# ajzhai/PEANUT

Hardware: AMD Instinct MI355X
Metric: maps/sec for 480x480x(4+N_cat) prediction fwd, batch 32 (higher is better)
Workload: dtype f32; 1 GPU; 480x480, 14-channel (4+10) partial maps -> 6-class prediction forward (PSPNet R50-V1c-D8), batch 32 per GPU, seeded random-init weights; survey_config=2, global_batch=32, parallelism=dp1 (map shards, no data-path collective)

## Files before the change

peanut_amd/csrc/options.h:

```cpp
#pragma once
#include <stdlib.h>
#include <string.h>

#include <string>

namespace peanut {

enum OptionId {
  OPT_PW_GLDS, OPT_PW256_MINK, OPT_PW256_MINTILES, OPT_PW256_PHASE, OPT_PW256_SKIP_PAD, OPT_PW256W_MINK, OPT_PW256W_MINTILES, OPT_PW256P_MINK, OPT_PW256P_MINTILES, OPT_PW256P_FLUSH, OPT_PW256P_ORDER, OPT_PW256P_STREAMK, OPT_PW256WP_MINK, OPT_PW256WP_MINTILES, OPT_PW256WP_NPRE, OPT_PW256WP_STAGGER, OPT_PW_ARES, OPT_PW_SKINNY,
  OPT_PW_ARES_MINUNITS, OPT_PATCH_MINTILES, OPT_STEM_NCHW, OPT_BN64_MAXK, OPT_PW_BN64_MAXK, OPT_PW64_MAXTILES, OPT_FP32_BK, OPT_NCHUNK, OPT_RES_PREFETCH, OPT_SPLIT_MODEL,
  OPT_RS_CONV, OPT_RS_BN64_MAXK, OPT_RS256_MINK, OPT_RS256_MINTILES, OPT_RS64_MAXK, OPT_RS64_MAXTILES,
  OPT_WINO_M, OPT_WINO_HEAD_M, OPT_WINO6_MAXDIL, OPT_WINO5_MINDIL, OPT_WINO_FLUSH_CH, OPT_WINO_MIN_CIN, OPT_WINO_NARROW_MINPIX, OPT_WINO_SMALL_MAXWG, OPT_DEFER_SPLITK,
  OPT_PPM_OVERLAP, OPT_PPM_GROUPED, OPT_PPM_TERM_ROWS, OPT_PPM_GROUP_ROWS, OPT_RCNN_WINO_M, OPT_RCNN_STEM_S2D, OPT_RCNN_RPN_FUSED, OPT_RCNN_FPN_OVERLAP, OPT_RCNN_RANK_SORT, OPT_RCNN_TOPK_SLICE, OPT_RCNN_NMS_LEVELS, OPT_FMM_LOCAL32, OPT_FMM_MAX_PASSES, OPT_FMM_BLOCKED, OPT_FMM_INNER,
  OPT_COUNT
};

struct OptionInfo {
  const char* key;
  long long def;
  bool upload_time;
  const char* help;
};

inline const OptionInfo* option_table() {
  static const OptionInfo t[OPT_COUNT] = {
      {"pw_glds", 1, false, "fp32 1x1 convs / grouped GEMMs on the LDS-DMA kernels of conv_pw.hip (0: conv_igemm)"},
      {"pw256_mink", 1024, false, "fewest input channels for the 256 x 128 three-stage kernel"},
      {"pw256_mintiles", 256, false, "fewest 256 x 128 tiles for that kernel"},
      {"pw256_phase", 1, false, "the two waves of a SIMD request their LDS-DMA pieces half an iteration apart"},
      {"pw256_skip_pad", 1, false, "256 x 128 kernel, grouped GEMMs: waves whose rows are all group padding issue no MFMAs (0: compute the zero rows)"},
      {"pw256w_mink", 768, false, "fewest input channels for the 256 x 256 two-stage kernel (0: off)"},
      {"pw256w_mintiles", 1536, false, "fewest 256 x 256 tiles for that kernel"},
      {"pw256p_mink", 512, false, "fewest input channels for the persistent 256 x 128 kernel (conv_pw256p.hip; 0: off)"},
      {"pw256p_mintiles", 512, false, "fewest 256 x 128 tiles for that kernel"},
      {"pw256p_flush", 512, false, "most input channels of a Winograd position GEMM (two-level accumulation) that runs on the persistent kernel (0: none)"},
      {"pw256p_order", 1, false, "persistent 256 x 128 kernel: 1 = the workgroups of an XCD walk its run of tiles side by side (neighbours share operand panels in L2), 0 = one contiguous run per workgroup"},
      {"pw256p_streamk", 1, false, "persistent 256 x 128 kernel: the tail tiles' k-tiles as one stream in equal runs per workgroup (0: every tail tile cut into the same number of parts)"},
      {"pw256wp_mink", 512, false, "fewest input channels for the persistent 256 x 256 kernel (conv_pw256wp.hip; 0: off)"},
      {"pw256wp_mintiles", 768, false, "fewest 256 x 256 tiles for that kernel"},
      {"pw256wp_npre", 0, false, "persistent 256 x 256 kernel: accumulator blocks per in-place epilogue group (2 or 4; 0 = two with a residual, four without)"},
      {"pw256wp_stagger", 0, false, "persistent 256 x 256 kernel: spread of the workgroups' start times in sleeps of ~3.4 us (their tile boundaries -- 512 KiB of epilogue traffic per CU -- then fall at different times)"},
      {"pw_ares", 1, false, "K = 128 / 256 pointwise layers on the persistent A-resident kernel (conv_pw_ares.hip)"},
      {"pw_skinny", 1, false, "grouped pointwise launches with at most 64 data rows per group (the PSP pyramid's per-scale convs and Q tables at batch 1) on the skinny weight-streaming kernel (gemm_skinny.hip: 6 KiB of LDS, fits next to any other kernel; 0: the MFMA kernels on 128-row padded tiles)"},
      {"pw_ares_minunits", 512, false, "fewest (m-tile, n-tile) units for that kernel"},
      {"patch_mintiles", 1024, false, "3x3 convs of 16 / 32 input channels on the persistent LDS-patch kernel (conv_patch.hip) from this many 8 x 16 output tiles (0: off)"},
      {"stem_nchw", 1, false, "prediction forward: the first stem conv reads the NCHW input itself (conv_patch.hip, NCHW variant) instead of a layout pass + NHWC conv (fp32 mode, when the patch kernel takes the layer)"},
      {"bn64_maxk", 256, true, "128 x 64 tiles for layers with at most this many input channels"},
      {"pw_bn64_maxk", 128, true, "pointwise layers / Winograd position GEMMs: weights PACKED 64 wide up to this many input channels (wider layers: 128-wide packing, 64-wide tiles chosen per shape)"},
      {"pw64_maxtiles", 512, false, "a 128-wide-packed pointwise layer with at most bn64_maxk input channels runs 128 x 64 tiles while its 128 x 128 tiling has fewer tiles than this (two per CU)"},
      {"fp32_bk", 0, true, "16: force 16-channel k-tiles in conv_igemm (experiment)"},
      {"nchunk", 8, false, "n-tiles per chunk of the tile order (0: n fastest over all n-tiles)"},
      {"res_prefetch", 1, false, "request the first residual rows before the last k-tile's MFMAs"},
      {"split_model", 1, false, "tail split-K plan counts CUs (1) or resident slots (0)"},
      {"rs_conv", 1, true, "emulated modes: non-pointwise convs on conv_rs.hip (0: fp32 MFMA kernel)"},
      {"rs_bn64_maxk", 128, true, "emulated modes: 128 x 64 tiles up to this many input channels"},
      {"rs256_mink", 512, false, "emulated modes: fewest input channels for the 256 x 256 kernel"},
      {"rs256_mintiles", 256, false, "emulated modes: fewest 256 x 256 tiles for it"},
      {"rs64_maxk", 512, false, "emulated modes: 64 x 64 tiles up to this many input channels"},
      {"rs64_maxtiles", 128, false, "emulated modes: ... and below this many 128-row tiles"},
      {"wino_m", 0, true, "4 / 5 / 6: force one Winograd form on every eligible layer (0: policy)"},
      {"wino_head_m", 0, true, "4 / 5 / 6: Winograd form of the PSP bottleneck (0: policy)"},
      {"wino6_maxdil", 4, true, "largest dilation that gets an F(6x6) form"},
      {"wino5_mindil", 4, true, "smallest dilation that also gets an F(5x5) form (0: none)"},
      {"wino_flush_ch", 64, true, "channels per partial sum of the position GEMMs' two-level accumulation (0: off)"},
      {"wino_min_cin", 0, true, "fewest input channels of a Winograd layer (0: the planner's policy)"},
      {"wino_narrow_minpix", 20000, false, "layers under 128 channels take their Winograd form from this many input pixels on (round 6: 100 000 -> 20 000 -- with the small-problem transforms one 720 x 720 map's layer1 conv2, 32 400 pixels, gains 5 us per layer as F(6x6); profiles/r9e)"},
      {"wino_small_maxwg", 1024, false, "Winograd transforms: launches with fewer workgroups than this of the one-thread-per-tile kernels take the small-problem variants (a workgroup per tile and 64-channel slice, a thread per line, through LDS; bit-identical; 0: never)"},
      {"defer_splitk", 1, false, "a Bottleneck conv1 whose every tile is split along k leaves its partial tiles unsummed and conv2's (small-problem) Winograd input transform sums them: one launch fewer per block at batch 1, bit-identical (0: every conv runs its own reduce); read when a (B, H, W) plan is built"},
      {"ppm_overlap", -1, false, "pyramid branch of the PSP head on a side stream: 0 / 1, -1 = by size"},
      {"ppm_grouped", -1, false, "per-scale PSP GEMMs as one grouped launch: 0 / 1, -1 = by size"},
      {"ppm_term_rows", 1, false, "folded pyramid term: one wave per output row, no barrier in the row loop (0: the workgroup-wide two-phase kernel)"},
      {"ppm_group_rows", 0, false, "pyramid pooling, row pass: rows added up per workgroup (1..5; 0 = by size: as many as still leave ~768 workgroups)"},
      {"rcnn_wino_m", 0, true, "detector front end: 4 / 5 / 6 pins one Winograd form (0: per shape)"},
      {"rcnn_stem_s2d", 1, true, "detector stem 7x7 stride 2 as a space-to-depth 4x4 conv"},
      {"rcnn_rpn_fused", 1, false, "detector: the RPN head on all five pyramid levels as one chain (five input transforms, ONE grouped Winograd GEMM, five output transforms, one objectness and one anchor-delta GEMM over all levels' rows: 12 launches instead of 25); read when a (B, H, W) plan is built"},
      {"rcnn_fpn_overlap", 0, false, "detector: the FPN output convs of p5, p4, p3 on a side stream next to the lateral / top-down chain that ends in p2's (round 5 experiment, bit-identical; measured SLOWER at batch 1, 5.70 against 5.61 ms per frame, profiles/r8: off); read when a (B, H, W) plan is built"},
      {"rcnn_rank_sort", 1, false, "detector: the RPN candidates of an image are ordered by counting the larger keys (n / 64 workgroups) instead of one workgroup's bitonic sort (round 5; same order: the keys are distinct)"},
      {"rcnn_topk_slice", 20480, false, "detector: objectness logits per workgroup of the per-level top-k (a level is cut into up to 8 ranges whose k largest are merged by counting; 0: one workgroup per level, round 4)"},
      {"rcnn_nms_levels", 1, false, "detector: the proposal NMS level by level (five 16 x 16-word suppression blocks and five scans per image side by side, post-NMS top-k by counting) instead of one score-sorted list per image (round 5; same proposals)"},
      {"fmm_local32", 1, false, "goal solver: single-precision local solve inside a tile"},
      {"fmm_max_passes", 24, false, "goal solver: hard ceiling of the second-order ordering passes; they stop as soon as a pass changes nothing (6-10 passes on the agent's 960 x 960 map; peanut_goal_converged reports whether they reached their fixed point)"},
      {"fmm_blocked", 1, false, "goal solver: a wave relaxes its 8 x 8 block of the tile to convergence between workgroup barriers (round 5; 0: one Jacobi sweep of the whole tile per barrier pair)"},
      {"fmm_inner", 48, false, "goal solver: iterations a wave spends on its block before it publishes it (blocked rounds)"},
  };
  return t;
}

struct Options {
  long long v[OPT_COUNT];
};

inline int option_index(const char* key) {
  if (!key) return -1;
  std::string k(key);
  for (auto& c : k) c = (char)((c >= 'A' && c <= 'Z') ? c - 'A' + 'a' : c);
  if (k.rfind("peanut_", 0) == 0) k = k.substr(7);
  const OptionInfo* t = option_table();
  for (int i = 0; i < OPT_COUNT; ++i)
    if (k == t[i].key) return i;
  return -1;
}

inline Options& default_options() {
  static Options d = [] {
    Options o;
    const OptionInfo* t = option_table();
    for (int i = 0; i < OPT_COUNT; ++i) {
      o.v[i] = t[i].def;
      std::string env = "PEANUT_";
      for (const char* c = t[i].key; *c; ++c) env += (char)((*c >= 'a' && *c <= 'z') ? *c - 'a' + 'A' : *c);
      const char* e = getenv(env.c_str());
      if (e && *e) o.v[i] = atoll(e);
    }
    return o;
  }();
  return d;
}

inline const Options*& active_options_ptr() {
  static thread_local const Options* p = nullptr;
  return p;
}

inline long long opt(OptionId id) {
  const Options* a = active_options_ptr();
  return (a ? a : &default_options())->v[id];
}

struct OptionScope {
  const Options* saved;
  explicit OptionScope(const Options* o) : saved(active_options_ptr()) { active_options_ptr() = o; }
  ~OptionScope() { active_options_ptr() = saved; }
  OptionScope(const OptionScope&) = delete;
  OptionScope& operator=(const OptionScope&) = delete;
};

}
```

peanut_amd/csrc/pred_api.hip:

```cpp
#include <math.h>
#include <string.h>

#include <map>
#include <memory>
#include <string>
#include <vector>

#include "net_common.h"

namespace peanut {

static thread_local std::string g_err;
void set_error(const std::string& msg) { g_err = msg; }
int fail(int code, const std::string& msg) {
  g_err = msg;
  return code;
}
static thread_local const char* g_kernel = "";
void note_kernel(const char* family) { g_kernel = family; }
const char* noted_kernel() { return g_kernel; }

namespace {

enum OpKind { OP_TO_NHWC, OP_CONV, OP_CONV_NCHW, OP_MAXPOOL, OP_PPM_POOL, OP_PPM_UP, OP_PPM_TERM, OP_UPSAMPLE, OP_WINO_IN, OP_WINO_GEMM, OP_WINO_OUT };

struct Op {
  OpKind kind;
  std::string name;
  std::string kernel;
  const ConvLayer* conv = nullptr;
  Act in, in2, res, out;
  bool has_in2 = false, has_res = false;
  double flops = 0;
  double bytes = 0;
  int wino_mt_per_group = 0;
  int wino_valid_rows = 0;
  int wino_gran = 128;
  int branch = 0;
  bool fork_before = false, join_before = false;
  int group_mt = 0;
  int ppm_scale_rows = 0;
  bool defer_ok = false;
};

struct Plan {
  int B = 0, H = 0, W = 0;
  Act splitk;
  Act splitk2;
  bool keep_all = false;
  size_t bytes = 0;
  std::vector<Op> ops;
  std::map<std::string, Act> named;
};

}
}

using namespace peanut;

struct peanut_conv {
  Options opts = default_options();
  ConvLayer L;
  DevBuf ws;
  DevBuf wino_v, wino_m;
};

struct peanut_pred {
  Options opts = default_options();
  DeferredSplit deferred{};
  peanut_pred_cfg cfg{};
  int cin_pad = 0;
  std::vector<std::unique_ptr<ConvLayer>> convs;
  ConvLayer* stem[3] = {nullptr, nullptr, nullptr};
  struct Block { ConvLayer *c1, *c2, *c3, *down, *c3d; };
  std::vector<std::vector<Block>> layers;
  std::vector<ConvLayer*> ppm;
  ConvLayer* bottleneck = nullptr;
  ConvLayer* bottleneck_x = nullptr;
  std::vector<ConvLayer*> ppm_q;
  std::unique_ptr<ConvLayer> ppm_grouped, ppmq_grouped;
  ConvLayer* conv_seg = nullptr;
  int feat_channels = 0;
  bool keep_all = false;
  std::map<std::string, std::unique_ptr<Plan>> plans;
  Plan* last_plan = nullptr;
  DevBuf ws;
  bool use_graph = false;
  GraphCache graphs;
  bool probe = false;
  Plan* probe_plan = nullptr;
  std::vector<std::vector<hipEvent_t>> probe_events;
  std::vector<hipEvent_t> event_pool;
  hipStream_t side = nullptr;
  hipEvent_t ev_fork = nullptr, ev_join = nullptr;
  ~peanut_pred() {
    for (auto& v : probe_events) for (auto e : v) (void)hipEventDestroy(e);
    for (auto e : event_pool) (void)hipEventDestroy(e);
    if (ev_fork) (void)hipEventDestroy(ev_fork);
    if (ev_join) (void)hipEventDestroy(ev_join);
    if (side) (void)hipStreamDestroy(side);
  }
};

namespace {

int bn_fold(peanut_pred* h, const TensorMap& tm, const std::string& bn, int cout, float* scale, float* shift) {
  return bn_fold_eps(tm, bn, cout, h->cfg.bn_eps, scale, shift);
}

int add_conv(peanut_pred* h, const TensorMap& tm, const std::string& conv, const std::string& bn, int cin,
             int cin_pad, int cout, int k, int stride, int pad, int dil, int relu, ConvLayer** out) {
  int rc = 0;
  const int64_t wshape[4] = {cout, cin, k, k};
  const peanut_tensor* w = tm.get(conv + ".weight", 4, wshape, &rc);
  if (!w) return rc;
  std::vector<float> scale(cout, 1.f), shift(cout, 0.f);
  const int64_t cshape[1] = {cout};
  if (!bn.empty()) {
    if ((rc = bn_fold(h, tm, bn, cout, scale.data(), shift.data()))) return rc;
  } else {
    const peanut_tensor* b = tm.get(conv + ".bias", 1, cshape, &rc); if (!b) return rc;
    for (int n = 0; n < cout; ++n) shift[n] = b->data[n];
  }
  auto L = std::make_unique<ConvLayer>();
  L->name = conv;
  rc = upload_conv(*L, w->data, scale.data(), shift.data(), cout, cin, cin_pad, k, k, stride, pad, dil, relu,
                   h->cfg.precision);
  if (rc) return rc;
  if (h->cfg.conv_algo == PEANUT_ALGO_AUTO && wino_eligible(cin_pad, cout, k, k, stride, pad, dil, h->cfg.precision, 64) &&
      (rc = upload_wino_forms(*L, w->data, scale.data(), shift.data(), cout, cin, cin_pad, pad, dil, relu, h->cfg.precision, 0)))
    return rc;
  *out = L.get();
  h->convs.push_back(std::move(L));
  return 0;
}

int add_fused_c3d(peanut_pred* h, const TensorMap& tm, const std::string& blk, int planes, int inplanes, int cout, ConvLayer** out) {
  int rc = 0;
  const int64_t w3s[4] = {cout, planes, 1, 1}, wds[4] = {cout, inplanes, 1, 1};
  const peanut_tensor* w3 = tm.get(blk + ".conv3.weight", 4, w3s, &rc);
  if (!w3) return rc;
  const peanut_tensor* wd = tm.get(blk + ".downsample.0.weight", 4, wds, &rc);
  if (!wd) return rc;
  std::vector<float> s3(cout), b3(cout), sd(cout), bd(cout);
  if ((rc = bn_fold(h, tm, blk + ".bn3", cout, s3.data(), b3.data()))) return rc;
  if ((rc = bn_fold(h, tm, blk + ".downsample.1", cout, sd.data(), bd.data()))) return rc;
  const int cin = planes + inplanes;
  std::vector<float> w((size_t)cout * cin), shift(cout);
  for (int n = 0; n < cout; ++n) {
    for (int c = 0; c < planes; ++c) w[(size_t)n * cin + c] = s3[n] * w3->data[(size_t)n * planes + c];
    for (int c = 0; c < inplanes; ++c) w[(size_t)n * cin + planes + c] = sd[n] * wd->data[(size_t)n * inplanes + c];
    shift[n] = b3[n] + bd[n];
  }
  auto L = std::make_unique<ConvLayer>();
  L->name = blk + ".conv3+downsample";
  if ((rc = upload_conv(*L, w.data(), nullptr, shift.data(), cout, cin, cin, 1, 1, 1, 0, 1, 1,
                        rs_planes_of(h->cfg.precision) ? h->cfg.precision : PEANUT_PREC_FP32))) return rc;
  *out = L.get();
  h->convs.push_back(std::move(L));
  return 0;
}

std::unique_ptr<ConvLayer> build_grouped(const std::vector<ConvLayer*>& parts, const std::string& name, int* rc) {
  *rc = 0;
  if (parts.size() < 2) return nullptr;
  const ConvDesc& d0 = parts[0]->d;
  for (const ConvLayer* L : parts)
    if (L->d.kh != 1 || L->d.kw != 1 || L->d.cin != d0.cin || L->d.cout != d0.cout || L->d.bn_tile != d0.bn_tile ||
        L->d.bk != d0.bk || L->d.relu != d0.relu || L->w.bytes != parts[0]->w.bytes || L->ss.bytes != parts[0]->ss.bytes)
      return nullptr;
  auto G = std::make_unique<ConvLayer>();
  G->name = name;
  G->d = d0;
  G->cin_real = parts[0]->cin_real;
  const size_t wb = parts[0]->w.bytes, sb = (size_t)d0.cout_pad * sizeof(float), n = parts.size();
// ... 119 lines not shown
      pl->ops.push_back(op);
    } else {
      push_conv(*pl, h->stem[i], x, nullptr, nullptr, y);
    }
    pl->named["stem" + std::to_string(i)] = y;
    if (!(i == 0 && nchw_stem)) rel(x);
    x = y;
  }
  {
    Act y = make_act(ar, B, conv_out_dim(x.H, 3, 2, 1, 1), conv_out_dim(x.W, 3, 2, 1, 1), x.C);
    Op op; op.kind = OP_MAXPOOL; op.name = "maxpool"; op.kernel = "maxpool"; op.in = x; op.out = y;
    op.bytes = (double)x.bytes + (double)y.bytes;
    pl->ops.push_back(op);
    pl->named["pool"] = y;
    rel(x);
    x = y;
  }
  for (size_t li = 0; li < h->layers.size(); ++li) {
    for (size_t bi = 0; bi < h->layers[li].size(); ++bi) {
      const auto& blk = h->layers[li][bi];
      const ConvDesc& d2 = blk.c2->d;
      Act t1 = make_act(ar, B, x.H, x.W, blk.c1->d.cout);
      push_conv(*pl, blk.c1, x, nullptr, nullptr, t1);
      const int h2 = conv_out_dim(x.H, 3, d2.stride, d2.pad, d2.dil), w2 = conv_out_dim(x.W, 3, d2.stride, d2.pad, d2.dil);
      Act t2 = make_act(ar, B, h2, w2, d2.cout);
      const size_t c1_idx = pl->ops.size() - 1;
      push_conv(*pl, blk.c2, t1, nullptr, nullptr, t2, &ar);
      {
        const Op& win = pl->ops[c1_idx + 1];
        if (opt(OPT_DEFER_SPLITK) != 0 && !h->keep_all && win.kind == OP_WINO_IN && pl->ops[c1_idx].kind == OP_CONV && !win.conv->d.rs &&
            wino_input_accepts_deferred(t1.B, t1.H, t1.W, t1.C, win.conv->d.dil, win.wino_gran, win.conv->wino_m))
          pl->ops[c1_idx].defer_ok = true;
      }
      rel(t1);
      Act idn = x;
      bool own_idn = false;
      const bool fused_c3d = blk.c3d != nullptr && !h->keep_all;
      if (blk.down && !fused_c3d) {
        idn = make_act(ar, B, h2, w2, blk.down->d.cout);
        push_conv(*pl, blk.down, x, nullptr, nullptr, idn);
        own_idn = true;
      }
      Act y = make_act(ar, B, h2, w2, blk.c3->d.cout);
      if (fused_c3d) push_conv(*pl, blk.c3d, t2, &x, nullptr, y);
      else push_conv(*pl, blk.c3, t2, nullptr, &idn, y);
      rel(t2);
      if (own_idn) rel(idn);
      rel(x);
      x = y;
    }
    pl->named["layer" + std::to_string(li + 1)] = x;
  }
  const int overlap_env = (int)opt(OPT_PPM_OVERLAP);
  const bool overlap = h->bottleneck_x != nullptr && (overlap_env >= 0 ? overlap_env == 1 : (long long)B * x.H * x.W >= 4096);
  const size_t side_first = pl->ops.size();
  if (overlap) {
    pl->splitk2.bytes = kSplitKScratchFloats * sizeof(float);
    pl->splitk2.off = ar.alloc(pl->splitk2.bytes);
    pl->splitk2.B = pl->splitk2.H = pl->splitk2.W = 1; pl->splitk2.C = 0;
  }
  std::vector<Act> side_bufs;
  auto rel_side = [&](const Act& t) { if (overlap) side_bufs.push_back(t); else rel(t); };
  int nbins = 0, kmax = 0;
  for (int i = 0; i < h->cfg.n_pool_scales; ++i) {
    nbins += h->cfg.pool_scales[i] * h->cfg.pool_scales[i];
    kmax = std::max(kmax, h->cfg.pool_scales[i]);
  }
  int srows = 0;
  if (h->ppm_grouped && h->ppmq_grouped && !h->keep_all) {
    const int cand = (B * kmax * kmax + 127) / 128 * 128;
    long long separate = 0;
    for (int i = 0; i < h->cfg.n_pool_scales; ++i) separate += ((long long)B * h->cfg.pool_scales[i] * h->cfg.pool_scales[i] + 127) / 128 * 128;
    const int env = (int)opt(OPT_PPM_GROUPED);
    if (env != 0 && ((long long)h->cfg.n_pool_scales * cand <= 2 * separate || env == 1)) srows = cand;
  }
  const int prow = srows ? h->cfg.n_pool_scales * srows : nbins * B;
  Act pooled = make_act(ar, 1, 1, prow, x.C);
  {
    Op op; op.kind = OP_PPM_POOL; op.name = "ppm_pool"; op.kernel = "ppm_pool"; op.in = x; op.out = pooled; op.ppm_scale_rows = srows;
    op.bytes = (double)x.bytes + (double)pooled.bytes;
    const size_t sf = ppm_pool_scratch_floats(B, x.H, x.C, h->cfg.pool_scales, h->cfg.n_pool_scales);
    if (sf) {
      Act scr; scr.B = 1; scr.H = 1; scr.W = 1; scr.C = 0; scr.bytes = sf * sizeof(float); scr.off = ar.alloc(scr.bytes);
      op.in2 = scr; op.has_in2 = true;
      pl->ops.push_back(op);
      rel_side(scr);
    } else {
      pl->ops.push_back(op);
    }
  }
  Act table = make_act(ar, 1, 1, prow, h->cfg.head_channels);
  auto push_grouped = [&](const ConvLayer* G, const Act& in, const Act& out) {
    push_conv(*pl, G, in, nullptr, nullptr, out);
    Op& op = pl->ops.back();
    op.group_mt = srows / 128;
    op.flops = 2.0 * (double)prow * G->d.cout * G->cin_real;
  };
  if (srows) {
    push_grouped(h->ppm_grouped.get(), pooled, table);
  } else {
    size_t row0 = 0;
    for (int i = 0; i < h->cfg.n_pool_scales; ++i) {
      const int k = h->cfg.pool_scales[i];
      Act in = pooled, out = table;
      in.off = pooled.off + row0 * (size_t)x.C * sizeof(float);
      in.H = 1; in.W = k * k; in.C = x.C; in.B = B;
      out.off = table.off + row0 * (size_t)h->cfg.head_channels * sizeof(float);
      out.H = 1; out.W = k * k; out.C = h->cfg.head_channels; out.B = B;
      push_conv(*pl, h->ppm[i], in, nullptr, nullptr, out);
      row0 += (size_t)B * k * k;
    }
  }
  pl->named["ppm_table"] = table;
  rel_side(pooled);
  Act bt;
  int term_scale_rows = 0;
  if (h->bottleneck_x) {
    const int hc = h->cfg.head_channels;
    Act q = make_act(ar, 1, 1, prow, 9 * hc);
    if (srows) {
      push_grouped(h->ppmq_grouped.get(), table, q);
      term_scale_rows = srows;
    } else {
      size_t row0 = 0;
      for (int i = 0; i < h->cfg.n_pool_scales; ++i) {
        const int k = h->cfg.pool_scales[i];
        Act in = table, out = q;
        in.off = table.off + row0 * (size_t)hc * sizeof(float);
        in.H = 1; in.W = k * k; in.C = hc; in.B = B;
        out.off = q.off + row0 * (size_t)(9 * hc) * sizeof(float);
        out.H = 1; out.W = k * k; out.C = 9 * hc; out.B = B;
        push_conv(*pl, h->ppm_q[i], in, nullptr, nullptr, out);
        row0 += (size_t)B * k * k;
      }
    }
    rel_side(table);
    Act r = make_act(ar, B, x.H, x.W, hc);
    {
      Op op; op.kind = OP_PPM_TERM; op.name = "ppm_conv_term"; op.kernel = "ppm_conv_term"; op.in = q; op.out = r; op.ppm_scale_rows = term_scale_rows;
      op.bytes = (double)q.bytes + (double)r.bytes;
      pl->ops.push_back(op);
    }
    rel_side(q);
    const size_t side_end = pl->ops.size();
    bt = make_act(ar, B, x.H, x.W, h->bottleneck_x->d.cout);
    push_conv(*pl, h->bottleneck_x, x, nullptr, &r, bt, &ar);
    if (overlap) {
      for (size_t i = side_first; i < side_end; ++i) pl->ops[i].branch = 1;
      pl->ops[side_first].fork_before = true;
      for (size_t i = side_end; i < pl->ops.size(); ++i)
        if (pl->ops[i].has_res) { pl->ops[i].join_before = true; break; }
      for (const auto& t : side_bufs) rel(t);
    }
    for (size_t i = side_first; i < side_end; ++i) {
      Op& op = pl->ops[i];
      if (op.kind == OP_CONV && op.group_mt == 1 && opt(OPT_PW_SKINNY) != 0 && B * kmax * kmax <= 64 &&
          op.conv->d.bn_tile == 128 && op.conv->d.bk == 32 && op.conv->d.cout % 128 == 0 && (op.conv->d.cin / 32) % 4 == 0)
        op.kernel = "gemm_skinny";
    }
    rel(r);
  } else {
    Act up = make_act(ar, B, x.H, x.W, h->cfg.n_pool_scales * h->cfg.head_channels);
    { Op op; op.kind = OP_PPM_UP; op.name = "ppm_upsample_concat"; op.kernel = "ppm_upsample_concat"; op.in = table; op.out = up; pl->ops.push_back(op); }
    rel(table);
    bt = make_act(ar, B, x.H, x.W, h->bottleneck->d.cout);
    push_conv(*pl, h->bottleneck, x, &up, nullptr, bt);
    rel(up);
  }
  pl->named["bottleneck"] = bt;
  rel(x);
  Act lo = make_act(ar, B, bt.H, bt.W, h->conv_seg->d.cout);
  push_conv(*pl, h->conv_seg, bt, nullptr, nullptr, lo);
  pl->named["logits_lowres"] = lo;
  rel(bt);
  {
    Op op; op.kind = OP_UPSAMPLE; op.name = "upsample_logits"; op.kernel = "upsample_logits"; op.in = lo;
    op.bytes = (double)lo.bytes + (double)B * H * W * h->conv_seg->d.cout * 4.0;
    pl->ops.push_back(op);
  }
  rel(lo);
  return pl;
}

}

static size_t plan_high_water(const Plan& pl) {
  size_t hw = 0;
  auto upd = [&](const Act& a) { if (a.bytes && a.off + Arena::round_up(a.bytes) > hw) hw = a.off + Arena::round_up(a.bytes); };
  for (const auto& op : pl.ops) {
    upd(op.in); upd(op.in2); upd(op.res); upd(op.out);
  }
  for (const auto& kv : pl.named) upd(kv.second);
  upd(pl.splitk);
  upd(pl.splitk2);
  return hw;
}

static Plan* get_plan(peanut_pred* h, int B, int H, int W) {
  if (B <= 0 || H < 16 || W < 16) { set_error("forward: need B >= 1 and H, W >= 16"); return nullptr; }
  const std::string key = std::to_string(B) + "x" + std::to_string(H) + "x" + std::to_string(W) + (h->keep_all ? "k" : "");
  auto it = h->plans.find(key);
  if (it == h->plans.end()) {
    auto pl = build_plan(h, B, H, W);
    pl->bytes = plan_high_water(*pl);
    it = h->plans.emplace(key, std::move(pl)).first;
  }
  return it->second.get();
}

static int run_op(peanut_pred* h, const Plan& pl, const Op& op, const float* in_dev, float* out_dev, int sigmoid,
                  hipStream_t s) {
  char* base = (char*)h->ws.p;
  auto P = [&](const Act& a) { return (float*)(base + a.off); };
  switch (op.kind) {
    case OP_TO_NHWC:
      return launch_nchw_to_nhwc_pad(in_dev, P(op.out), pl.B, h->cfg.in_channels, pl.H, pl.W, h->cin_pad, s);
    case OP_CONV_NCHW:
      return launch_conv_patch_nchw(op.conv->d, in_dev, h->cfg.in_channels, P(op.out), pl.B, pl.H, pl.W, op.out.H, op.out.W, s);
    case OP_CONV: {
      ConvArgs a{};
      a.x = P(op.in);
      a.x2 = op.has_in2 ? P(op.in2) : nullptr;
      a.res = op.has_res ? P(op.res) : nullptr;
      a.y = P(op.out);
      a.B = op.in.B; a.H = op.in.H; a.W = op.in.W;
      a.c1 = op.in.C; a.c2 = op.has_in2 ? op.in2.C : 0;
      a.Ho = op.out.H; a.Wo = op.out.W;
      a.ws = P(op.branch ? pl.splitk2 : pl.splitk); a.ws_floats = kSplitKScratchFloats;
      int scale_rows[8] = {0};
      if (op.group_mt) {
        int most = 0;
        for (int i = 0; i < h->cfg.n_pool_scales && i < 8; ++i) {
          scale_rows[i] = pl.B * h->cfg.pool_scales[i] * h->cfg.pool_scales[i];
          most = std::max(most, scale_rows[i]);
        }
        a.group_valid_rows = most;
        a.group_rows = scale_rows;
        a.mt_per_group = op.group_mt;
        a.w_group_stride = op.conv->w.bytes / sizeof(float) / (size_t)h->cfg.n_pool_scales;
        a.ss_group_stride = op.conv->d.cout_pad;
      }
      if (op.defer_ok) a.defer = &h->deferred;
      return launch_conv(op.conv->d, a, s);
    }
    case OP_WINO_IN: {
      const int rc = launch_wino_input(P(op.in), P(op.out), op.in.B, op.in.H, op.in.W, op.in.C, op.conv->d.dil, s, op.wino_gran, op.conv->wino_m, 0,
                                       h->deferred.valid ? &h->deferred : nullptr);
      h->deferred.valid = false;
      return rc;
    }
    case OP_WINO_GEMM: {
      ConvArgs a{};
      a.x = P(op.in); a.y = P(op.out);
      a.B = 1; a.H = 1; a.W = op.in.W; a.c1 = op.in.C; a.c2 = 0; a.Ho = 1; a.Wo = op.in.W;
      a.ws = P(op.branch ? pl.splitk2 : pl.splitk); a.ws_floats = kSplitKScratchFloats;
      a.mt_per_group = op.wino_mt_per_group;
      a.group_valid_rows = op.wino_valid_rows;
      a.w_group_stride = op.conv->wino.rs ? op.conv->wino_group_bytes : op.conv->wino_group_floats;
      return launch_conv(op.conv->wino, a, s);
    }
    case OP_WINO_OUT:
      return launch_wino_output(P(op.in), op.conv->d.scale, op.conv->d.shift, op.has_res ? P(op.res) : nullptr, P(op.out),
                                op.out.B, op.out.H, op.out.W, op.out.C, op.conv->d.dil, op.conv->d.relu, s, op.wino_gran, op.conv->wino_m);
    case OP_MAXPOOL:
      return launch_maxpool3x3s2(P(op.in), P(op.out), op.in.B, op.in.H, op.in.W, op.in.C, op.out.H, op.out.W, s);
    case OP_PPM_POOL:
      return launch_ppm_pool2(P(op.in), op.has_in2 ? P(op.in2) : nullptr, P(op.out), op.in.B, op.in.H, op.in.W, op.in.C,
                              h->cfg.pool_scales, h->cfg.n_pool_scales, s, op.ppm_scale_rows);
    case OP_PPM_UP:
      return launch_ppm_upsample_concat(P(op.in), P(op.out), op.out.B, op.out.H, op.out.W, h->cfg.head_channels,
                                        h->cfg.pool_scales, h->cfg.n_pool_scales, h->cfg.align_corners, s);
    case OP_PPM_TERM:
      return launch_ppm_conv_term(P(op.in), P(op.out), op.out.B, op.out.H, op.out.W, h->cfg.head_channels,
                                  h->cfg.pool_scales, h->cfg.n_pool_scales, h->cfg.align_corners, s, op.ppm_scale_rows);
    case OP_UPSAMPLE:
      return launch_upsample_logits(P(op.in), out_dev, op.in.B, op.in.H, op.in.W, op.in.C, pl.H, pl.W,
                                    h->cfg.align_corners, sigmoid, s);
  }
  return fail(PEANUT_EINVAL, "unknown op");
}

extern "C" {

const char* peanut_last_error(void) { return g_err.c_str(); }
const char* peanut_last_conv_kernel(void) { return noted_kernel(); }
int peanut_abi_version(void) { return 17; }
const char* peanut_build_arch(void) { return "gfx950"; }
#ifndef PEANUT_SOURCE_HASH
#define PEANUT_SOURCE_HASH ""
#endif
const char* peanut_source_hash(void) { return PEANUT_SOURCE_HASH; }

namespace {
int option_lookup(const char* key, const char* who) {
  const int i = option_index(key);
  if (i < 0) return fail(PEANUT_EINVAL, std::string(who) + ": unknown option '" + (key ? key : "(null)") + "'");
  return i;
}
int handle_set_option(Options& o, const char* key, long long value, const char* who) {
  const int i = option_lookup(key, who);
  if (i < 0) return i;
  if (option_table()[i].upload_time)
    return fail(PEANUT_EINVAL, std::string(who) + ": option '" + option_table()[i].key +
                                   "' shapes the uploaded weights; set it with peanut_set_default_option before creating the handle");
  o.v[i] = value;
  return 0;
}
}

int peanut_set_default_option(const char* key, long long value) {
  const int i = option_lookup(key, "peanut_set_default_option");
  if (i < 0) return i;
// ... 363 lines not shown
```

peanut_amd/csrc/pspnet_aux.hip:

```cpp
#include <algorithm>
#include <vector>

#include "common.h"
#include "options.h"

namespace peanut {

static inline unsigned grid_for(long long work_items, int block = 256) {
  long long g = (work_items + block - 1) / block;
  const long long cap = 256LL * 8;
  if (g > cap) g = cap;
  if (g < 1) g = 1;
  return (unsigned)g;
}

__global__ __launch_bounds__(256) void nchw_to_nhwc_pad_kernel(const float* __restrict__ x, float* __restrict__ y,
                                                               int C, long long HW, long long npix, int Cpad) {
  __shared__ float t[256][17];
  const long long p0 = (long long)blockIdx.x * 256;
  for (int c0 = 0; c0 < Cpad; c0 += 16) {
    const long long pix = p0 + threadIdx.x;
    if (pix < npix) {
      const long long b = pix / HW, hw = pix - b * HW;
      const float* src = x + (b * C) * HW + hw;
// ... 497 lines not shown
__global__ __launch_bounds__(64 * NW) void ppm_conv_term_rows_kernel(const float* __restrict__ Q, float* __restrict__ R,
                                                                     int H, int W, int C, PpmScales sc, int B, int nbins,
                                                                     int align_corners) {
  extern __shared__ __attribute__((aligned(16))) unsigned char lds_raw[];
  constexpr int CH = 32;
  float* q = reinterpret_cast<float*>(lds_raw);
  BlTap* taps = reinterpret_cast<BlTap*>(lds_raw + (size_t)nbins * 9 * CH * sizeof(float));
  const int L = (H > W ? H : W) + 2;
  const int b = blockIdx.y, c0 = blockIdx.x * CH;
  {
    int base = 0;
    for (int s = 0; s < sc.n; ++s) {
      const int k = sc.s[s], cells = k * k;
      const float* src = Q + (ppm_row0(sc, s, base, B) + (size_t)b * cells) * (9 * C) + c0;
      for (int i = threadIdx.x; i < cells * 9 * (CH / 4); i += blockDim.x) {
        const int v4 = i % (CH / 4), rt = i / (CH / 4);
        const float4 v = *reinterpret_cast<const float4*>(src + (size_t)rt * C + v4 * 4);
        *reinterpret_cast<float4*>(q + ((size_t)(base * 9 + rt)) * CH + v4 * 4) = v;
      }
      base += cells;
    }
  }
  for (int i = threadIdx.x; i < sc.n * 2 * L; i += blockDim.x) {
    const int s = i / (2 * L), r = i - s * 2 * L, dim = r / L, t = r - dim * L;
    const int n = dim == 0 ? H : W, coord = t - 1;
    BlTap tp;
    tp.i0 = -1; tp.i1 = -1; tp.l = 0.f;
    if ((unsigned)coord < (unsigned)n) {
      int i0, i1;
      float l;
      bilinear_src(coord, sc.s[s], n, align_corners, &i0, &i1, &l);
      tp.i0 = (short)i0; tp.i1 = (short)i1; tp.l = l;
    }
    taps[i] = tp;
  }
  __syncthreads();
  int slots = 0;
  for (int s = 0; s < sc.n; ++s) slots += sc.s[s];
  const int wave = threadIdx.x >> 6, lane = threadIdx.x & 63;
  float* srow = reinterpret_cast<float*>(taps + (size_t)sc.n * 2 * L) + (size_t)wave * slots * 3 * CH;
  const int rows_per = (H + gridDim.z - 1) / gridDim.z;
  const int y_begin = blockIdx.z * rows_per, y_end = min(H, y_begin + rows_per);
  for (int yy = y_begin + wave; yy < y_end; yy += NW) {
    for (int i = lane; i < slots * 3 * (CH / 4); i += 64) {
      const int g = i % (CH / 4), r = i / (CH / 4), dx = r % 3, slot = r / 3;
      int s = 0, gx = slot, base = 0;
      while (gx >= sc.s[s]) { gx -= sc.s[s]; base += sc.s[s] * sc.s[s]; ++s; }
      const int k = sc.s[s];
      const BlTap* ty = taps + (s * 2 + 0) * L + yy;
      const float* qs = q + (size_t)base * 9 * CH + g * 4;
      float4 acc = make_float4(0.f, 0.f, 0.f, 0.f);
#pragma unroll
      for (int dy = 0; dy < 3; ++dy) {
        const BlTap t = ty[dy];
        if (t.i0 < 0) continue;
        const float hy = 1.f - t.l;
        const float4 v0 = *reinterpret_cast<const float4*>(qs + ((t.i0 * k + gx) * 9 + dy * 3 + dx) * CH);
        const float4 v1 = *reinterpret_cast<const float4*>(qs + ((t.i1 * k + gx) * 9 + dy * 3 + dx) * CH);
        acc.x += hy * v0.x + t.l * v1.x; acc.y += hy * v0.y + t.l * v1.y;
        acc.z += hy * v0.z + t.l * v1.z; acc.w += hy * v0.w + t.l * v1.w;
      }
      *reinterpret_cast<float4*>(srow + (size_t)r * CH + g * 4) = acc;
    }
    asm volatile("s_waitcnt lgkmcnt(0)" ::: "memory");
    __builtin_amdgcn_wave_barrier();
    for (int it = lane; it < W * (CH / 4); it += 64) {
      const int g = it % (CH / 4), xx = it / (CH / 4);
      float4 acc = make_float4(0.f, 0.f, 0.f, 0.f);
      int slot0 = 0;
      for (int s = 0; s < sc.n; ++s) {
        const BlTap* tx = taps + (s * 2 + 1) * L + xx;
#pragma unroll
        for (int dx = 0; dx < 3; ++dx) {
          const BlTap t = tx[dx];
          if (t.i0 < 0) continue;
          const float hx = 1.f - t.l;
          const float4 v0 = *reinterpret_cast<const float4*>(srow + ((size_t)(slot0 + t.i0) * 3 + dx) * CH + g * 4);
          const float4 v1 = *reinterpret_cast<const float4*>(srow + ((size_t)(slot0 + t.i1) * 3 + dx) * CH + g * 4);
          acc.x += hx * v0.x + t.l * v1.x; acc.y += hx * v0.y + t.l * v1.y;
          acc.z += hx * v0.z + t.l * v1.z; acc.w += hx * v0.w + t.l * v1.w;
        }
        slot0 += sc.s[s];
      }
      *reinterpret_cast<float4*>(R + (((size_t)b * H + yy) * W + xx) * C + c0 + g * 4) = acc;
    }
    asm volatile("s_waitcnt lgkmcnt(0)" ::: "memory");
    __builtin_amdgcn_wave_barrier();
  }
}

int launch_ppm_conv_term(const float* Q, float* R, int B, int H, int W, int C, const int* scales, int nscales,
                         int align_corners, hipStream_t s, int scale_rows) {
  if (nscales <= 8 && C % 32 == 0) {
    PpmScales sc;
    sc.n = nscales;
    sc.rows = scale_rows;
    int nbins = 0;
    for (int i = 0; i < nscales; ++i) { sc.s[i] = scales[i]; nbins += scales[i] * scales[i]; }
    const int L = (H > W ? H : W) + 2;
    int slots = 0;
    for (int i = 0; i < nscales; ++i) slots += scales[i];
    const size_t lds = (size_t)nbins * 9 * 32 * sizeof(float) + (size_t)nscales * 2 * L * sizeof(BlTap) +
                       (size_t)slots * 3 * 32 * sizeof(float);
    constexpr int ROWS_NW = 16;
    const size_t lds_rows = lds + (size_t)(ROWS_NW - 1) * slots * 3 * 32 * sizeof(float);
    if (lds_rows <= 150 * 1024 && opt(OPT_PPM_TERM_ROWS) != 0 && (long long)(C / 32) * B >= 128) {
      static bool raised_rows = false;
      if (!raised_rows) {
        hipError_t e = hipFuncSetAttribute(reinterpret_cast<const void*>(ppm_conv_term_rows_kernel<ROWS_NW>),
                                           hipFuncAttributeMaxDynamicSharedMemorySize, 150 * 1024);
        if (e != hipSuccess) return fail(-3, std::string("hipFuncSetAttribute: ") + hipGetErrorString(e));
        raised_rows = true;
      }
      int row_splits = (256 + (C / 32) * B - 1) / ((C / 32) * B);
      row_splits = std::max(1, std::min(row_splits, H / ROWS_NW > 0 ? H / ROWS_NW : 1));
      hipLaunchKernelGGL(ppm_conv_term_rows_kernel<ROWS_NW>, dim3(C / 32, B, row_splits), dim3(64 * ROWS_NW), lds_rows, s, Q, R, H, W, C,
                         sc, B, nbins, align_corners);
      hipError_t e = hipGetLastError();
      return e == hipSuccess ? 0 : fail(-3, std::string("ppm_conv_term_rows: ") + hipGetErrorString(e));
    }
    if (lds <= 150 * 1024) {
      static bool raised = false;
      if (!raised) {
        hipError_t e = hipFuncSetAttribute(reinterpret_cast<const void*>(ppm_conv_term_lds_kernel),
                                           hipFuncAttributeMaxDynamicSharedMemorySize, 150 * 1024);
        if (e != hipSuccess) return fail(-3, std::string("hipFuncSetAttribute: ") + hipGetErrorString(e));
        raised = true;
      }
      int row_splits = (512 + (C / 32) * B - 1) / ((C / 32) * B);
      row_splits = std::max(1, std::min(row_splits, H / 4 > 0 ? H / 4 : 1));
      hipLaunchKernelGGL(ppm_conv_term_lds_kernel, dim3(C / 32, B, row_splits), dim3(256), lds, s, Q, R, H, W, C, sc, B, nbins,
                         align_corners);
      hipError_t e = hipGetLastError();
      return e == hipSuccess ? 0 : fail(-3, std::string("ppm_conv_term_lds: ") + hipGetErrorString(e));
    }
  }
  return launch_ppm_conv_term_l2(Q, R, B, H, W, C, scales, nscales, align_corners, s, scale_rows);
}

int launch_ppm_conv_term_l2(const float* Q, float* R, int B, int H, int W, int C, const int* scales, int nscales,
                            int align_corners, hipStream_t s, int scale_rows) {
  if (nscales > 8 || C % 4) return fail(-2, "ppm_conv_term: unsupported configuration");
  PpmScales sc;
  sc.n = nscales;
  sc.rows = scale_rows;
  for (int i = 0; i < nscales; ++i) sc.s[i] = scales[i];
  const long long total = (long long)B * H * W * (C / 4);
  hipLaunchKernelGGL(ppm_conv_term_kernel, dim3(grid_for(total)), dim3(256), 0, s, Q, R, H, W, C, sc, B,
                     align_corners, total);
  hipError_t e = hipGetLastError();
  return e == hipSuccess ? 0 : fail(-3, std::string("ppm_conv_term: ") + hipGetErrorString(e));
}

template <int KMAX>
__global__ __launch_bounds__(256) PEANUT_NO_PK_F32 void upsample_logits_kernel(const float* __restrict__ lo, float* __restrict__ out,
                                                              int h, int w, int K, int H, int W, int align_corners,
                                                              int sigmoid, long long total) {
  for (long long i = (long long)blockIdx.x * blockDim.x + threadIdx.x; i < total;
       i += (long long)gridDim.x * blockDim.x) {
    const int xx = (int)(i % W);
    const long long t = i / W;
    const int yy = (int)(t % H);
    const long long b = t / H;
    int y0, y1, x0, x1;
    float ly, lx;
    bilinear_src(yy, h, H, align_corners, &y0, &y1, &ly);
    bilinear_src(xx, w, W, align_corners, &x0, &x1, &lx);
    const float hy = 1.f - ly, hx = 1.f - lx;
    const float* p00 = lo + (((size_t)b * h + y0) * w + x0) * K;
    const float* p01 = lo + (((size_t)b * h + y0) * w + x1) * K;
    const float* p10 = lo + (((size_t)b * h + y1) * w + x0) * K;
    const float* p11 = lo + (((size_t)b * h + y1) * w + x1) * K;
    float* o = out + ((size_t)b * K) * H * W + (size_t)yy * W + xx;
#pragma unroll
    for (int k = 0; k < KMAX; ++k) {
      if (k < K) {
        float v = hy * (hx * p00[k] + lx * p01[k]) + ly * (hx * p10[k] + lx * p11[k]);
        if (sigmoid) v = 1.f / (1.f + expf(-v));
        o[(size_t)k * H * W] = v;
      }
    }
  }
}

int launch_upsample_logits(const float* lo, float* out, int B, int h, int w, int K, int H, int W,
                           int align_corners, int sigmoid, hipStream_t s) {
  const long long total = (long long)B * H * W;
  if (K <= 8)
    hipLaunchKernelGGL(upsample_logits_kernel<8>, dim3(grid_for(total)), dim3(256), 0, s, lo, out, h, w, K, H, W,
                       align_corners, sigmoid, total);
  else if (K <= 32)
    hipLaunchKernelGGL(upsample_logits_kernel<32>, dim3(grid_for(total)), dim3(256), 0, s, lo, out, h, w, K, H, W,
                       align_corners, sigmoid, total);
  else
    return fail(-2, "upsample_logits: more than 32 classes is not supported");
  hipError_t e = hipGetLastError();
  return e == hipSuccess ? 0 : fail(-3, std::string("upsample_logits: ") + hipGetErrorString(e));
}

}
```

Baseline: 893.3 maps/s.

## Add late PPM fork point and vectorize logits upsampling by four columns

Adds a ppm_fork option that can move the pyramid branch's side-stream fork to just after the bottleneck Winograd input transform, so that it overlaps the MFMA-bound position GEMM instead of another HBM-bound kernel. The default is 0, the existing fork point, so the rotation is inactive by default. Separately, the final logits upsample now has each thread produce four adjacent output columns. It reuses source pixels across those columns and writes 16-byte vector stores when W is divisible by 4 and the output is aligned. This cuts redundant loads and scalar stores in a large memory-bound output kernel, at the cost of more registers per thread.

Result: no change. 892.6 maps/s (median of 3 runs) (-0.1%).

```diff
diff --git a/peanut_amd/csrc/options.h b/peanut_amd/csrc/options.h
--- a/peanut_amd/csrc/options.h
+++ b/peanut_amd/csrc/options.h
@@ -11,7 +11,7 @@
   OPT_PW_ARES_MINUNITS, OPT_PATCH_MINTILES, OPT_STEM_NCHW, OPT_BN64_MAXK, OPT_PW_BN64_MAXK, OPT_PW64_MAXTILES, OPT_FP32_BK, OPT_NCHUNK, OPT_RES_PREFETCH, OPT_SPLIT_MODEL,
   OPT_RS_CONV, OPT_RS_BN64_MAXK, OPT_RS256_MINK, OPT_RS256_MINTILES, OPT_RS64_MAXK, OPT_RS64_MAXTILES,
   OPT_WINO_M, OPT_WINO_HEAD_M, OPT_WINO6_MAXDIL, OPT_WINO5_MINDIL, OPT_WINO_FLUSH_CH, OPT_WINO_MIN_CIN, OPT_WINO_NARROW_MINPIX, OPT_WINO_SMALL_MAXWG, OPT_DEFER_SPLITK,
-  OPT_PPM_OVERLAP, OPT_PPM_GROUPED, OPT_PPM_TERM_ROWS, OPT_PPM_GROUP_ROWS, OPT_RCNN_WINO_M, OPT_RCNN_STEM_S2D, OPT_RCNN_RPN_FUSED, OPT_RCNN_FPN_OVERLAP, OPT_RCNN_RANK_SORT, OPT_RCNN_TOPK_SLICE, OPT_RCNN_NMS_LEVELS, OPT_FMM_LOCAL32, OPT_FMM_MAX_PASSES, OPT_FMM_BLOCKED, OPT_FMM_INNER,
+  OPT_PPM_OVERLAP, OPT_PPM_FORK, OPT_PPM_GROUPED, OPT_PPM_TERM_ROWS, OPT_PPM_GROUP_ROWS, OPT_RCNN_WINO_M, OPT_RCNN_STEM_S2D, OPT_RCNN_RPN_FUSED, OPT_RCNN_FPN_OVERLAP, OPT_RCNN_RANK_SORT, OPT_RCNN_TOPK_SLICE, OPT_RCNN_NMS_LEVELS, OPT_FMM_LOCAL32, OPT_FMM_MAX_PASSES, OPT_FMM_BLOCKED, OPT_FMM_INNER,
   OPT_COUNT
 };
 
@@ -68,6 +68,7 @@
       {"wino_small_maxwg", 1024, false, "Winograd transforms: launches with fewer workgroups than this of the one-thread-per-tile kernels take the small-problem variants (a workgroup per tile and 64-channel slice, a thread per line, through LDS; bit-identical; 0: never)"},
       {"defer_splitk", 1, false, "a Bottleneck conv1 whose every tile is split along k leaves its partial tiles unsummed and conv2's (small-problem) Winograd input transform sums them: one launch fewer per block at batch 1, bit-identical (0: every conv runs its own reduce); read when a (B, H, W) plan is built"},
       {"ppm_overlap", -1, false, "pyramid branch of the PSP head on a side stream: 0 / 1, -1 = by size"},
+      {"ppm_fork", 0, false, "two-stream PSP head: where the pyramid branch forks: 0 = before ppm_pool (next to the bottleneck's Winograd input transform, both HBM-bound), 1 = behind that transform (next to the MFMA-bound position GEMM), -1 = by size (1 from 16 384 bottleneck pixels on); bit-identical; read when a (B, H, W) plan is built"},
       {"ppm_grouped", -1, false, "per-scale PSP GEMMs as one grouped launch: 0 / 1, -1 = by size"},
       {"ppm_term_rows", 1, false, "folded pyramid term: one wave per output row, no barrier in the row loop (0: the workgroup-wide two-phase kernel)"},
       {"ppm_group_rows", 0, false, "pyramid pooling, row pass: rows added up per workgroup (1..5; 0 = by size: as many as still leave ~768 workgroups)"},
diff --git a/peanut_amd/csrc/pred_api.hip b/peanut_amd/csrc/pred_api.hip
--- a/peanut_amd/csrc/pred_api.hip
+++ b/peanut_amd/csrc/pred_api.hip
@@ -1,6 +1,7 @@
 #include <math.h>
 #include <string.h>
 
+#include <algorithm>
 #include <map>
 #include <memory>
 #include <string>
@@ -21,6 +22,8 @@
 const char* noted_kernel() { return g_kernel; }
 
 namespace {
+
+constexpr long long kPpmForkLateRows = 16384;
 
 enum OpKind { OP_TO_NHWC, OP_CONV, OP_CONV_NCHW, OP_MAXPOOL, OP_PPM_POOL, OP_PPM_UP, OP_PPM_TERM, OP_UPSAMPLE, OP_WINO_IN, OP_WINO_GEMM, OP_WINO_OUT };
 
@@ -446,12 +449,19 @@
         if (pl->ops[i].has_res) { pl->ops[i].join_before = true; break; }
       for (const auto& t : side_bufs) rel(t);
     }
+    bool fork_late = false;
+    if (overlap && side_end < pl->ops.size() && pl->ops[side_end].kind == OP_WINO_IN) {
+      const int fk = (int)opt(OPT_PPM_FORK);
+      fork_late = fk >= 0 ? fk == 1 : (long long)B * x.H * x.W >= kPpmForkLateRows;
+    }
     for (size_t i = side_first; i < side_end; ++i) {
       Op& op = pl->ops[i];
       if (op.kind == OP_CONV && op.group_mt == 1 && opt(OPT_PW_SKINNY) != 0 && B * kmax * kmax <= 64 &&
           op.conv->d.bn_tile == 128 && op.conv->d.bk == 32 && op.conv->d.cout % 128 == 0 && (op.conv->d.cin / 32) % 4 == 0)
         op.kernel = "gemm_skinny";
     }
+    if (fork_late)
+      std::rotate(pl->ops.begin() + side_first, pl->ops.begin() + side_end, pl->ops.begin() + side_end + 1);
     rel(r);
   } else {
     Act up = make_act(ar, B, x.H, x.W, h->cfg.n_pool_scales * h->cfg.head_channels);
diff --git a/peanut_amd/csrc/pspnet_aux.hip b/peanut_amd/csrc/pspnet_aux.hip
--- a/peanut_amd/csrc/pspnet_aux.hip
+++ b/peanut_amd/csrc/pspnet_aux.hip
@@ -673,10 +673,61 @@
   return e == hipSuccess ? 0 : fail(-3, std::string("ppm_conv_term: ") + hipGetErrorString(e));
 }
 
-template <int KMAX>
+typedef float up_f32x4 __attribute__((ext_vector_type(4)));
+template <int KMAX, int VX>
 __global__ __launch_bounds__(256) PEANUT_NO_PK_F32 void upsample_logits_kernel(const float* __restrict__ lo, float* __restrict__ out,
                                                               int h, int w, int K, int H, int W, int align_corners,
                                                               int sigmoid, long long total) {
+  const size_t plane = (size_t)H * W;
+  if constexpr (VX == 4) {
+    const unsigned W4 = (unsigned)W >> 2, n = (unsigned)total;
+    for (unsigned i = blockIdx.x * 256u + threadIdx.x; i < n; i += gridDim.x * 256u) {
+      const unsigned t = i / W4;
+      const int xx0 = (int)(i - t * W4) * 4;
+      const unsigned b = t / (unsigned)H;
+      const int yy = (int)(t - b * (unsigned)H);
+      int y0, y1;
+      float ly;
+      bilinear_src(yy, h, H, align_corners, &y0, &y1, &ly);
+      const float hy = 1.f - ly;
+      const float* r0 = lo + ((size_t)b * h + y0) * w * K;
+      const float* r1 = lo + ((size_t)b * h + y1) * w * K;
+      float* o = out + ((size_t)b * K) * plane + (size_t)yy * W + xx0;
+      float a00[KMAX], a01[KMAX], a10[KMAX], a11[KMAX], res[KMAX][4];
+      int px0 = -1, px1 = -1;
+#pragma unroll
+      for (int j = 0; j < 4; ++j) {
+        int x0, x1;
+        float lx;
+        bilinear_src(xx0 + j, w, W, align_corners, &x0, &x1, &lx);
+        const float hx = 1.f - lx;
+        if (x0 != px0 || x1 != px1) {
+          const float* p00 = r0 + (size_t)x0 * K;
+          const float* p01 = r0 + (size_t)x1 * K;
+          const float* p10 = r1 + (size_t)x0 * K;
+          const float* p11 = r1 + (size_t)x1 * K;
+#pragma unroll
+          for (int k = 0; k < KMAX; ++k) {
+            if (k < K) { a00[k] = p00[k]; a01[k] = p01[k]; a10[k] = p10[k]; a11[k] = p11[k]; }
+          }
+          px0 = x0; px1 = x1;
+        }
+#pragma unroll
+        for (int k = 0; k < KMAX; ++k) {
+          if (k < K) {
+            float v = hy * (hx * a00[k] + lx * a01[k]) + ly * (hx * a10[k] + lx * a11[k]);
+            if (sigmoid) v = 1.f / (1.f + expf(-v));
+            res[k][j] = v;
+          }
+        }
+      }
+#pragma unroll
+      for (int k = 0; k < KMAX; ++k) {
+        if (k < K) *reinterpret_cast<up_f32x4*>(o + (size_t)k * plane) = up_f32x4{res[k][0], res[k][1], res[k][2], res[k][3]};
+      }
+    }
+    return;
+  }
   for (long long i = (long long)blockIdx.x * blockDim.x + threadIdx.x; i < total;
        i += (long long)gridDim.x * blockDim.x) {
     const int xx = (int)(i % W);
@@ -707,11 +758,15 @@
 int launch_upsample_logits(const float* lo, float* out, int B, int h, int w, int K, int H, int W,
                            int align_corners, int sigmoid, hipStream_t s) {
   const long long total = (long long)B * H * W;
-  if (K <= 8)
-    hipLaunchKernelGGL(upsample_logits_kernel<8>, dim3(grid_for(total)), dim3(256), 0, s, lo, out, h, w, K, H, W,
+  const bool vx4 = K <= 8 && W % 4 == 0 && ((uintptr_t)out & 15) == 0 && total / 4 < (1LL << 31) - 256LL * 64 * 256;
+  if (vx4)
+    hipLaunchKernelGGL((upsample_logits_kernel<8, 4>), dim3(grid_for(total / 4)), dim3(256), 0, s, lo, out, h, w, K, H, W,
+                       align_corners, sigmoid, total / 4);
+  else if (K <= 8)
+    hipLaunchKernelGGL((upsample_logits_kernel<8, 1>), dim3(grid_for(total)), dim3(256), 0, s, lo, out, h, w, K, H, W,
                        align_corners, sigmoid, total);
   else if (K <= 32)
-    hipLaunchKernelGGL(upsample_logits_kernel<32>, dim3(grid_for(total)), dim3(256), 0, s, lo, out, h, w, K, H, W,
+    hipLaunchKernelGGL((upsample_logits_kernel<32, 1>), dim3(grid_for(total)), dim3(256), 0, s, lo, out, h, w, K, H, W,
                        align_corners, sigmoid, total);
   else
     return fail(-2, "upsample_logits: more than 32 classes is not supported");
```
